# X-rayLaser/Implementing-JPEG-compression

Hardware: AMD Instinct MI355X
Metric: M 8x8 blocks/sec (DCT+quant+zigzag) (higher is better)
Workload: dtype f32

## Files before the change

implementing-jpeg-compression_amd/csrc/jpegx_entropy_decode.h:

```cpp
#pragma once
#include <hip/hip_runtime.h>
#include <stddef.h>
#include <stdint.h>

namespace jpegx_decode {
int levels_for(long long nblocks);
size_t phase1_bytes(size_t nbytes);
size_t phase2_bytes(size_t ncand, long long nblocks);
void enqueue_phase1(const uint8_t *d_bytes, size_t nbytes, void *d_ws1, hipStream_t st);
void enqueue_phase2(const uint8_t *d_bytes, size_t nbytes, long long nblocks, void *d_ws1, unsigned ncand, void *d_ws2,
                    int16_t *d_zz, hipStream_t st);

struct SegPlan {
    int seg, cmax, levels;
    int span_cap;
    unsigned nseg;
    size_t ws_bytes, state_bytes;
    bool ok;
    bool filter;
};
SegPlan seg_plan(size_t nbytes, long long nblocks, int level = 0, int filter = -1);
void enqueue_segmented(const uint8_t *d_bytes, size_t nbytes, long long nblocks, const SegPlan &plan, void *d_state, size_t state_cap, bool fresh, int parity,
                       void *d_ws, int16_t *d_zz, hipStream_t st);
}
```

implementing-jpeg-compression_amd/csrc/jpegx_entropy_decode.hip:

```cpp
#include <hip/hip_runtime.h>
#include <stdint.h>
#include <stdlib.h>

#include "../../include/jpegx.h"
#include "jpegx_entropy_decode.h"

namespace {

typedef unsigned u32x4 __attribute__((ext_vector_type(4)));
constexpr unsigned NIL = 0xFFFFFFFFu;
constexpr int CHUNK = 4096;
__device__ __forceinline__ int tile_off(int row, int chunk) { return row * 128 + ((chunk ^ (row & 7)) << 4); }

__device__ __forceinline__ unsigned zero_mask16(const unsigned char *__restrict__ bytes, size_t q0, size_t nbytes)
{
    unsigned m = 0;
    if (q0 + 16 <= nbytes) {
        const u32x4 v = *reinterpret_cast<const u32x4 *>(bytes + q0);
        const unsigned w[4] = {v.x, v.y, v.z, v.w};
#pragma unroll
        for (int k = 0; k < 16; ++k) m |= (((w[k >> 2] >> (8 * (k & 3))) & 0xFFu) == 0u ? 1u : 0u) << k;
    } else {
        for (int k = 0; k < 16; ++k)
            if (q0 + k < nbytes && bytes[q0 + k] == 0) m |= 1u << k;
    }
    return m;
}

__global__ __launch_bounds__(256) void k_dec_count(const unsigned char *__restrict__ bytes, size_t nbytes, unsigned *__restrict__ chunk_count)
{
    __shared__ unsigned part[4];
    const size_t q0 = (size_t)blockIdx.x * CHUNK + (size_t)threadIdx.x * 16;
    unsigned c = q0 < nbytes ? __popc(zero_mask16(bytes, q0, nbytes)) : 0u;
    if (blockIdx.x == 0 && threadIdx.x == 0) c += 1;
#pragma unroll
// ... 152 lines not shown

__device__ __forceinline__ void dec_blocks_body(const unsigned *__restrict__ words, size_t nbytes, const unsigned *__restrict__ start_pos,
                                                int nblk, int16_t *__restrict__ out, unsigned *__restrict__ head)
{
    __shared__ __attribute__((aligned(16))) unsigned char lds[64 * 128];
    const int lane = threadIdx.x, g0 = blockIdx.x * 64, g = g0 + lane;
#pragma unroll
    for (int c = 0; c < 8; ++c) *reinterpret_cast<u32x4 *>(lds + lane * 128 + c * 16) = u32x4{0u, 0u, 0u, 0u};
    __syncthreads();
    if (g < nblk) {
        const unsigned p = start_pos[g];
        const unsigned e = p == NIL ? NIL : parse_block<true>(words, (unsigned long long)nbytes * 8u, p, lds, lane);
        if (e == NIL) atomicOr(&head[1], 2u);
        else if (g == nblk - 1 && e != (unsigned)nbytes) atomicOr(&head[1], 4u);
    }
    __syncthreads();
    unsigned char *dst = reinterpret_cast<unsigned char *>(out) + (size_t)g0 * 128;
#pragma unroll
    for (int i = 0; i < 8; ++i) {
        const int row = i * 8 + (lane >> 3), c = lane & 7;
        const u32x4 q = *reinterpret_cast<const u32x4 *>(lds + tile_off(row, c));
        if (g0 + row < nblk) *reinterpret_cast<u32x4 *>(dst + (size_t)row * 128 + c * 16) = q;
    }
}

__global__ __launch_bounds__(64) void k_dec_blocks(const unsigned *__restrict__ words, size_t nbytes, const unsigned *__restrict__ start_pos,
                                                   int nblk, int16_t *__restrict__ out, unsigned *__restrict__ head)
{
    dec_blocks_body(words, nbytes, start_pos, nblk, out, head);
}

namespace seg {

typedef __attribute__((address_space(1))) unsigned gu32;
#define JPEGX_RLX_AGENT __ATOMIC_RELAXED, __HIP_MEMORY_SCOPE_AGENT

constexpr int REACH = 192;
constexpr int ROW = 144;
constexpr int FRONT = 16, TAIL = 208;
constexpr unsigned INVALID = 0xFFFFu, END = 0xFFFEu, AFTER = 0xFFFDu, POISON = 0xFFFCu, EXIT = 0x8000u;
constexpr unsigned TAG = 0x10000u;
constexpr unsigned SPIN_LIMIT = 1u << 18;
__device__ __forceinline__ bool is_exit(unsigned x) { return (x & EXIT) != 0 && x < POISON; }

struct Ws {
    unsigned *head;
    unsigned *next_head;
    unsigned *E;
    unsigned *C;
    unsigned *F;
    unsigned *wave_seg;
    u32x4 *prov;
    unsigned long long *trace;
};

__host__ __device__ inline size_t up16(size_t v) { return (v + 15) & ~(size_t)15; }

__host__ __device__ inline Ws carve(void *state, void *scratch, unsigned nseg, int cmax, long long nblocks, int parity, size_t *scratch_bytes = nullptr,
                                    size_t *state_bytes = nullptr)
{
    unsigned char *q = static_cast<unsigned char *>(state), *p = static_cast<unsigned char *>(scratch);
    Ws w;
    w.head = reinterpret_cast<unsigned *>(q + 64 * parity);
    w.next_head = reinterpret_cast<unsigned *>(q + 64 * (1 - parity));
    w.E = reinterpret_cast<unsigned *>(q + 128);
    if (state_bytes) *state_bytes = 128 + up16((size_t)nseg * 4);
    size_t o = 0;
    w.C = reinterpret_cast<unsigned *>(p + o); o += up16((size_t)nseg * 4 + 64);
    w.F = reinterpret_cast<unsigned *>(p + o); o += up16(((size_t)nseg + 1) * 4);
    w.wave_seg = reinterpret_cast<unsigned *>(p + o); o += up16((size_t)((nblocks + 63) / 64) * 4);
    w.prov = reinterpret_cast<u32x4 *>(p + o); o += up16((size_t)nseg * cmax * 16);
    w.trace = reinterpret_cast<unsigned long long *>(p + o);
#ifdef JPEGX_DECODE_STATS
    o += 64 + (size_t)nseg * 128;
#endif
    if (scratch_bytes) *scratch_bytes = o;
    return w;
}

__host__ __device__ inline int levels_of(int cmax)
{
    int l = 0;
    while ((1 << l) < cmax) ++l;
    return l;
}

__host__ __device__ inline size_t dec_lds_bytes(int span_cap) { return (size_t)span_cap + 64 * ROW + 1024 + 288; }

__host__ __device__ inline size_t lds_bytes(int seg, int cmax)
{
    return (size_t)(FRONT + seg + TAIL) + 64 * 12 + 256 + (size_t)cmax * (4 + levels_of(cmax));
}

constexpr int MARK_STEPS = 5;

__device__ __forceinline__ void fill_advance_table(unsigned char *tab, int lane)
{
    unsigned packed = 0;
#pragma unroll
// ... 76 lines not shown
    const size_t readable = (nbytes + 16) & ~(size_t)3;
    u32x4 v[PER];
#pragma unroll
    for (int k = 0; k < PER; ++k) {
        const int i = lane + THREADS * k;
        const long long off = first_off + 16LL * i;
        v[k] = u32x4{0u, 0u, 0u, 0u};
        if (i < npieces) {
            if (off >= 0 && (size_t)off + 16 <= readable) {
                v[k] = *reinterpret_cast<const u32x4 *>(bytes + off);
            } else {
                unsigned t[4] = {0u, 0u, 0u, 0u};
#pragma unroll
                for (int j = 0; j < 4; ++j) {
                    const long long o = off + 4 * j;
                    if (o >= 0 && (size_t)o + 4 <= readable) t[j] = *reinterpret_cast<const unsigned *>(bytes + o);
                }
                v[k] = u32x4{t[0], t[1], t[2], t[3]};
            }
        }
    }
#pragma unroll
    for (int k = 0; k < PER; ++k) {
        const int i = lane + THREADS * k;
        if (i < npieces) {
            u32x4 b = v[k];
            b.x = __builtin_bswap32(b.x); b.y = __builtin_bswap32(b.y); b.z = __builtin_bswap32(b.z); b.w = __builtin_bswap32(b.w);
            *reinterpret_cast<u32x4 *>(sm + 16 * i) = b;
        }
    }
}

__global__ __launch_bounds__(64) void k_seg_starts(const unsigned char *__restrict__ bytes, size_t nbytes, int seg, int cmax, unsigned nseg,
                                                   void *state, void *ws, long long nblocks, int parity, int filter)
{
    extern __shared__ __attribute__((aligned(16))) unsigned char sm[];
    const Ws W = carve(state, ws, nseg, cmax, nblocks, parity);
    gu32 *gE = (gu32 *)W.E;
    gu32 *ghead = (gu32 *)W.head;
    const int lane = threadIdx.x;
    const unsigned s = xcd_run_segment(blockIdx.x);
    if (s >= nseg) return;
#ifdef JPEGX_DECODE_STATS
    unsigned long long *trace = W.trace + 8 + (size_t)s * 16;
    if (lane == 0) trace[0] = wall_clock64();
    if (lane == 0 && s == 0) { unsigned *info = reinterpret_cast<unsigned *>(W.trace); info[4] = nseg; info[5] = (unsigned)seg; info[6] = (unsigned)cmax; info[7] = (unsigned)nblocks; }
#define JPEGX_PHASE(k) do { if (lane == 0) trace[(k) + 1] = wall_clock64(); } while (0)
#else
#define JPEGX_PHASE(k) do { } while (0)
#endif
    const int win = FRONT + seg + TAIL;
    const int levels = levels_of(cmax);
    unsigned *sw = reinterpret_cast<unsigned *>(sm);
    struct LaneRec { unsigned lo, hi, front; };
    LaneRec *rec = reinterpret_cast<LaneRec *>(sm + win);
    unsigned char *tab = reinterpret_cast<unsigned char *>(rec + 64);
    unsigned short *cpos = reinterpret_cast<unsigned short *>(tab + 256);
    unsigned short *J = cpos + cmax;
    unsigned char *Jk = reinterpret_cast<unsigned char *>(J + cmax) - cmax;

    const size_t base = (size_t)s * seg;
    stage_pieces<5>(bytes, nbytes, (long long)base - FRONT, win / 16, sm, lane);
    fill_advance_table(tab, lane);
    __syncthreads();
    JPEGX_PHASE(0);

    const int stretch = seg >> 6;
    const unsigned inv = ((1u << 20) + (unsigned)stretch - 1u) / (unsigned)stretch;
    const int p0 = lane * stretch;
    unsigned long long m;
    {
        const unsigned *swl = reinterpret_cast<const unsigned *>(sm + FRONT + p0);
// ... 20 lines not shown
        }
    }
    const unsigned mine = (unsigned)__popcll(m);
    unsigned incl = mine;
#pragma unroll
    for (int d = 1; d < 64; d <<= 1) {
        const unsigned u = (unsigned)__shfl_up((int)incl, d);
        if (lane >= d) incl += u;
    }
    const unsigned total = (unsigned)__shfl((int)incl, 63);
    rec[lane] = LaneRec{(unsigned)m, (unsigned)(m >> 32), incl - mine};
    const bool overflow = total > (unsigned)cmax;
    if (!overflow) {
        unsigned at = incl - mine;
        unsigned long long mm = m;
        while (mm) {
            const int i = __ffsll((long long)mm) - 1;
            mm &= mm - 1;
            cpos[at++] = (unsigned short)(p0 + i);
        }
    }
    __syncthreads();
    auto rank_of = [&](unsigned p, bool &is_cand) -> unsigned {
        const unsigned L = (p * inv) >> 20;
        const unsigned bit = p - L * (unsigned)stretch;
        const LaneRec r = rec[L];
        const unsigned long long mk = ((unsigned long long)r.hi << 32) | r.lo;
        is_cand = ((mk >> bit) & 1ull) != 0;
        return r.front + (unsigned)__popcll(mk & ((1ull << bit) - 1ull));
    };
    JPEGX_PHASE(1);

    bool poisoned = overflow;
    if (overflow && lane == 0) __hip_atomic_fetch_or(ghead + 2, 1u, JPEGX_RLX_AGENT);
    const size_t win_end = nbytes - base + FRONT;
    const unsigned end_bits = (unsigned)((win_end < (size_t)(win - 16) ? win_end : (size_t)(win - 16)) * 8u);
    unsigned nent = 0;
    bool konst = false;
    int lv = 1;
    while ((1u << (lv - 1)) < total && lv < levels) ++lv;
    auto chase = [&](unsigned c, unsigned &blocks) -> unsigned {
        unsigned cur = c, cnt = 0;
        for (int k = lv - 1; k >= 1; --k) {
            const unsigned nxt = Jk[k * cmax + cur];
            if (nxt != 0xFFu) { cur = nxt; cnt += 1u << k; }
        }
        const unsigned nxt0 = J[cur];
        if (nxt0 < EXIT) { cur = nxt0; cnt += 1u; }
        blocks = cnt + 1u;
        return J[cur];
    };
    unsigned my_exit_if_entry = INVALID, my_blocks_if_entry = 0;
    unsigned marks[2][3] = {{0u, 0u, 0u}, {0u, 0u, 0u}};
    if (!poisoned) {
        for (unsigned c0 = 0; c0 < total; c0 += 64) {
            const unsigned c = c0 + lane;
            const bool have = c < total;
            const unsigned p = have ? cpos[c] : 0u;
            unsigned mk[3];
            const unsigned e = parse_tab(sw, tab, (FRONT + p) * 8u, end_bits, have, mk);
#pragma unroll
            for (int k = 0; k < 3; ++k) {
                if (c0 == 0) marks[0][k] = mk[k];
                if (c0 == 64) marks[1][k] = mk[k];
            }
            unsigned code = INVALID;
            if (e != NIL) {
// ... 3 lines not shown
                else {
                    bool is_cand;
                    const unsigned i = rank_of(er, is_cand);
                    code = is_cand ? i : INVALID;
                }
            }
            if (have) J[c] = (unsigned short)code;
        }
        __syncthreads();
        JPEGX_PHASE(2);
        for (int k = 1; k < lv; ++k) {
            for (unsigned c = lane; c < total; c += 64) {
                unsigned two = 0xFFu;
                if (k == 1) {
                    const unsigned a = J[c];
                    if (a < EXIT) { const unsigned b = J[a]; if (b < EXIT) two = b; }
                } else {
                    const unsigned a = Jk[(k - 1) * cmax + c];
                    if (a != 0xFFu) two = Jk[(k - 1) * cmax + a];
                }
                Jk[k * cmax + c] = (unsigned char)two;
            }
            __syncthreads();
        }
        bool dummy_b;
        nent = total ? rank_of(REACH + 1, dummy_b) : 0u;
        if ((unsigned)lane < nent) my_exit_if_entry = chase((unsigned)lane, my_blocks_if_entry);
        if (nent >= 1 && nent <= 64) {
            const unsigned x = my_exit_if_entry;
            const unsigned long long valid = __ballot(x != INVALID);
            if (valid) {
                const unsigned x0 = (unsigned)__shfl((int)x, __ffsll((long long)valid) - 1);
                konst = __ballot(x != INVALID && x != x0) == 0;
                if (konst && lane == 0) __hip_atomic_store(gE + s, TAG | x0, JPEGX_RLX_AGENT);
            }
        }
    }
    JPEGX_PHASE(3);

    unsigned entry = INVALID, myexit = INVALID, count = 0, err = 0;
    if (!poisoned) {
        if (s == 0) {
            entry = total ? 0u : INVALID;
        } else {
            unsigned x = 0;
            unsigned dbg_spins = 0;
            for (unsigned spins = 0;;) {
                x = __hip_atomic_load(gE + (s - 1), JPEGX_RLX_AGENT);
                if (x != 0) break;
                ++dbg_spins;
                if (++spins > SPIN_LIMIT) { poisoned = true; break; }
                __builtin_amdgcn_s_sleep(2);
            }
            x &= 0xFFFFu;
            (void)dbg_spins;
#ifdef JPEGX_DECODE_STATS
            if (lane == 0) trace[12] = dbg_spins;
#endif
            if (poisoned || x == POISON) poisoned = true;
            else if (x == END || x == AFTER) entry = AFTER;
            else if (is_exit(x)) {
                const unsigned rel = x & 0x7FFFu;
                bool is_cand = false;
                const unsigned i = rel < (unsigned)seg ? rank_of(rel, is_cand) : 0u;
                entry = is_cand ? i : INVALID;
            }
        }
    }
    JPEGX_PHASE(4);
    if (!poisoned) {
        if (entry == AFTER) myexit = AFTER;
        else if (entry == INVALID) err |= filter ? 0x100u : 2u;
        else {
            if (entry < 64u && entry < nent) {
                myexit = (unsigned)__shfl((int)my_exit_if_entry, (int)entry);
                count = (unsigned)__shfl((int)my_blocks_if_entry, (int)entry);
            } else {
                myexit = chase(entry, count);
            }
            if (myexit == INVALID) { err |= filter ? 0x100u : 2u; count = 0; }
        }
        if ((err & 0xFFu) && lane == 0) __hip_atomic_fetch_or(ghead + 1, err & 0xFFu, JPEGX_RLX_AGENT);
        if ((err & 0x100u) && lane == 0) __hip_atomic_fetch_or(ghead + 2, 4u, JPEGX_RLX_AGENT);
        for (unsigned r0 = 0; r0 < count; r0 += 64) {
            const unsigned r = r0 + lane;
            unsigned cur = entry;
            if (r < count) {
                if (r & 1u) cur = J[cur];
                for (int k = 1; k < lv; ++k)
                    if ((r >> k) & 1u) cur = Jk[k * cmax + cur];
            }
            unsigned mk[3];
#pragma unroll
            for (int k = 0; k < 3; ++k) {
                const unsigned a = (unsigned)__shfl((int)marks[0][k], (int)(cur & 63u)), b = (unsigned)__shfl((int)marks[1][k], (int)(cur & 63u));
                mk[k] = cur < 64u ? a : (cur < 128u ? b : 0u);
            }
            if (r < count) W.prov[(size_t)s * cmax + r] = u32x4{(unsigned)base + cpos[cur], mk[0], mk[1], mk[2]};
        }
    } else if (lane == 0) {
        __hip_atomic_fetch_or(ghead + 2, 2u, JPEGX_RLX_AGENT);
    }
    if (lane == 0) {
        if (poisoned) __hip_atomic_store(gE + s, TAG | POISON, JPEGX_RLX_AGENT);
        else if (!konst || myexit == INVALID) __hip_atomic_store(gE + s, TAG | myexit, JPEGX_RLX_AGENT);
        W.C[s] = count;
    }
#ifdef JPEGX_DECODE_STATS
    if (lane == 0) { trace[15] = total; trace[13] = konst ? 1 : 0; trace[14] = count; }
#endif
    JPEGX_PHASE(5);
}

__global__ __launch_bounds__(1024) void k_seg_scan(unsigned nseg, int cmax, void *state, void *ws, long long nblocks, int parity)
{
    __shared__ unsigned carry[16];
    __shared__ unsigned base_s;
    const Ws W = carve(state, ws, nseg, cmax, nblocks, parity);
    const int t = threadIdx.x, lane = t & 63, wv = t >> 6;
    const unsigned nwaves = (unsigned)((nblocks + 63) / 64);
    if (t == 0) base_s = 0;
    __syncthreads();
    for (unsigned c0 = 0; c0 < nseg; c0 += 16384u) {
        const unsigned i0 = c0 + (unsigned)t * 16u;
        unsigned c[16];
        if (i0 + 16u <= nseg) {
#pragma unroll
            for (int k = 0; k < 4; ++k) {
                const u32x4 v = *reinterpret_cast<const u32x4 *>(W.C + i0 + 4 * k);
                c[4 * k] = v.x; c[4 * k + 1] = v.y; c[4 * k + 2] = v.z; c[4 * k + 3] = v.w;
            }
        } else {
#pragma unroll
            for (int k = 0; k < 16; ++k) c[k] = i0 + k < nseg ? W.C[i0 + k] : 0u;
        }
        unsigned sum = 0;
#pragma unroll
        for (int k = 0; k < 16; ++k) sum += c[k];
        unsigned incl = sum;
#pragma unroll
        for (int d = 1; d < 64; d <<= 1) {
            const unsigned u = (unsigned)__shfl_up((int)incl, d);
            if (lane >= d) incl += u;
        }
        if (lane == 63) carry[wv] = incl;
        __syncthreads();
        unsigned run = base_s + incl - sum;
        for (int k = 0; k < wv; ++k) run += carry[k];
#pragma unroll
        for (int k = 0; k < 16; ++k) {
            const unsigned i = i0 + k;
            if (i < nseg) {
                W.F[i] = run;
                for (unsigned m = (run + 63u) & ~63u; m < run + c[k]; m += 64)
                    if ((m >> 6) < nwaves) W.wave_seg[m >> 6] = i;
            }
            run += c[k];
        }
        __syncthreads();
        if (t == 1023) base_s = run;
        __syncthreads();
    }
    if (t == 0) {
        const unsigned run = base_s;
        W.F[nseg] = run;
        W.head[3] = run;
        unsigned err = 0;
        if ((long long)run < nblocks) err |= 1u;
        if ((long long)run > nblocks) err |= 4u;
        if (err) atomicOr(&W.head[1], err);
    }
}

__global__ __launch_bounds__(256) void k_dec_blocks_lds(const unsigned char *__restrict__ bytes, size_t nbytes, unsigned nseg, int cmax, void *state,
                                                        const void *ws, int nblk, int span_cap, int16_t *__restrict__ out, int parity)
{
    extern __shared__ __attribute__((aligned(16))) unsigned char sm[];
    const Ws W = carve(state, const_cast<void *>(ws), nseg, cmax, nblk, parity);
    for (unsigned i = blockIdx.x * 256u + threadIdx.x; i < nseg; i += gridDim.x * 256u) W.E[i] = 0u;
    if (blockIdx.x == 0 && threadIdx.x < 16) W.next_head[threadIdx.x] = 0u;
    const unsigned s0 = W.wave_seg[blockIdx.x], refused = W.head[1], handed_on = W.head[2];
    if (refused != 0 || handed_on != 0) return;
    const int t = threadIdx.x, lane = t & 63, part = t >> 6;
    const int tile_idx = blockIdx.x, g0 = tile_idx * 64, g = g0 + lane;
#ifdef JPEGX_DECODE_STATS
    unsigned long long *trace3 = W.trace + 8 + (size_t)tile_idx * 16;
    if (t == 0 && (unsigned)tile_idx < nseg) trace3[7] = wall_clock64();
#define JPEGX_PHASE3(k) do { if (t == 0 && (unsigned)tile_idx < nseg) trace3[k] = wall_clock64(); } while (0)
#else
#define JPEGX_PHASE3(k) do { } while (0)
#endif
    unsigned char *tile = sm + span_cap;
    unsigned char *dummy = tile + 64 * ROW + t * 4;
    unsigned *Fs = reinterpret_cast<unsigned *>(tile + 64 * ROW + 1024);
    for (int i = t; i < 64 * ROW / 16; i += 256) *reinterpret_cast<u32x4 *>(tile + i * 16) = u32x4{0u, 0u, 0u, 0u};
    if (t <= 64) Fs[t] = s0 + t <= nseg ? W.F[s0 + t] : 0xFFFFFFFFu;
    __syncthreads();
    auto entry_of = [&](unsigned blk) -> u32x4 {
        unsigned lo = 0, hi = 65;
        while (hi - lo > 1) {
            const unsigned mid = (lo + hi) >> 1;
            if (Fs[mid] <= blk) lo = mid; else hi = mid;
        }
        unsigned sgm = s0 + lo, first = Fs[lo];
        if (lo == 64) {
            unsigned a = s0 + 64, b = nseg;
            while (b - a > 1) {
                const unsigned mid = a + ((b - a) >> 1);
                if (W.F[mid] <= blk) a = mid; else b = mid;
            }
            sgm = a; first = W.F[a];
        }
        return W.prov[(size_t)sgm * cmax + (blk - first)];
// ... 74 lines not shown
    const char *force = getenv("JPEGX_DECODE_SEG");
    if (force && *force) k = atoi(force) / 256;
    if (level >= 1) k = 1;
    k = k < 1 ? 1 : (k > 16 ? 16 : k);
    if (level == 0 && !(force && *force)) {
        static const int ncu = [] { int v = 0, dev = 0; if (hipGetDevice(&dev) != hipSuccess || hipDeviceGetAttribute(&v, hipDeviceAttributeMultiprocessorCount, dev) != hipSuccess || v <= 0) v = 256; return v; }();
        const int cmax_l0 = p.filter ? 96 : 128;
        auto margin = [&](int kk) {
            const size_t lds = (seg::lds_bytes(256 * kk, cmax_l0) + 1279) / 1280 * 1280;
            const size_t per_cu = 163840 / lds > 32 ? 32 : 163840 / lds;
            const double slots = (double)ncu * (double)per_cu, waves = (double)((nbytes + 256 * (size_t)kk - 1) / (256 * (size_t)kk));
            return 1.0 - waves / slots;
        };
        if (margin(k) < 0.03) {
            int best = k;
            double best_margin = 0.03;
            for (int kk : {k + 1, k - 1, k + 2, k - 2})
                if (kk >= 1 && kk <= 16 && per_byte * 256.0 * kk <= 56.0 && margin(kk) > best_margin) { best = kk; best_margin = margin(kk); }
            k = best;
        }
    }
    p.seg = 256 * k;
    p.cmax = p.filter ? 96 : 128;
    const char *fc = getenv("JPEGX_DECODE_CMAX");
    if (fc && *fc) { p.cmax = atoi(fc); p.cmax = p.cmax < 32 ? 32 : (p.cmax > 128 ? 128 : p.cmax); }
    p.levels = seg::levels_of(p.cmax);
    p.nseg = (unsigned)((nbytes + p.seg - 1) / p.seg);
    size_t span = (size_t)(per_block * 64.0 * 1.5) + 64;
    span = (span + 15) & ~(size_t)15;
    if (span < 1024) span = 1024;
    if (span > 64 * 185 + 48) span = 64 * 185 + 48;
    p.span_cap = (int)span;
    p.ok = nbytes > 0 && (size_t)p.nseg * p.cmax * 16 <= ((size_t)1 << 32) && nblocks > 0;
    seg::carve(nullptr, nullptr, p.nseg ? p.nseg : 1, p.cmax, nblocks > 0 ? nblocks : 1, 0, &p.ws_bytes, &p.state_bytes);
    return p;
}

void enqueue_segmented(const uint8_t *d_bytes, size_t nbytes, long long nblocks, const SegPlan &p, void *d_state, size_t state_cap, bool fresh, int parity,
                       void *d_ws, int16_t *d_zz, hipStream_t st)
{
    if (fresh) (void)hipMemsetAsync(d_state, 0, state_cap, st);
#ifdef JPEGX_DECODE_STATS
    (void)hipMemsetAsync(d_ws, 0, p.ws_bytes, st);
#endif
    const unsigned run8 = 8u << seg::RUN_LOG;
    hipLaunchKernelGGL(seg::k_seg_starts, dim3((p.nseg + run8 - 1) / run8 * run8), dim3(64), seg::lds_bytes(p.seg, p.cmax), st, d_bytes, nbytes, p.seg, p.cmax,
                       p.nseg, d_state, d_ws, nblocks, parity, p.filter ? 1 : 0);
    hipLaunchKernelGGL(seg::k_seg_scan, dim3(1), dim3(1024), 0, st, p.nseg, p.cmax, d_state, d_ws, nblocks, parity);
    hipLaunchKernelGGL(seg::k_dec_blocks_lds, dim3((unsigned)((nblocks + 63) / 64)), dim3(256), seg::dec_lds_bytes(p.span_cap), st, d_bytes, nbytes,
                       p.nseg, p.cmax, d_state, d_ws, (int)nblocks, p.span_cap, d_zz, parity);
}

size_t phase1_bytes(size_t nbytes) { return 64 + ((nbytes + CHUNK - 1) / CHUNK + 1) * 4; }

size_t phase2_bytes(size_t ncand, long long nblocks)
{
    return ((size_t)ncand * 4 + 15) / 16 * 16 + (size_t)levels_for(nblocks) * ncand * 4 + (size_t)nblocks * 4 + 64;
}

void enqueue_phase1(const uint8_t *d_bytes, size_t nbytes, void *d_ws1, hipStream_t st)
{
    unsigned *head = static_cast<unsigned *>(d_ws1);
    unsigned *chunk = head + 4;
    const int nchunks = (int)((nbytes + CHUNK - 1) / CHUNK);
    (void)hipMemsetAsync(head, 0, 16, st);
    hipLaunchKernelGGL(k_dec_count, dim3(nchunks), dim3(256), 0, st, d_bytes, nbytes, chunk);
    hipLaunchKernelGGL(k_dec_scan, dim3(1), dim3(1024), 0, st, chunk, nchunks, head);
}

void enqueue_phase2(const uint8_t *d_bytes, size_t nbytes, long long nblocks, void *d_ws1, unsigned ncand, void *d_ws2,
                    int16_t *d_zz, hipStream_t st)
{
    unsigned *head = static_cast<unsigned *>(d_ws1);
    unsigned *chunk = head + 4;
    unsigned *cand_pos = static_cast<unsigned *>(d_ws2);
    unsigned *J = cand_pos + ((size_t)ncand * 4 + 15) / 16 * 4;
    const int levels = levels_for(nblocks);
    unsigned *start_pos = J + (size_t)levels * ncand;
    const unsigned *words = reinterpret_cast<const unsigned *>(d_bytes);
    const int nchunks = (int)((nbytes + CHUNK - 1) / CHUNK);
    const unsigned gc = (ncand + 255) / 256;
    hipLaunchKernelGGL(k_dec_scatter, dim3(nchunks), dim3(256), 0, st, d_bytes, nbytes, chunk, cand_pos);
    hipLaunchKernelGGL(k_dec_parse, dim3(gc), dim3(256), 0, st, words, nbytes, cand_pos, ncand, J);
// ... 9 lines not shown
```

implementing-jpeg-compression_amd/csrc/jpegx_hostpipe.cpp:

```cpp
#include <hip/hip_runtime.h>
#include <stdint.h>
#include <stdio.h>
#include <stdlib.h>
#include <string.h>
#include <time.h>
#include <sys/mman.h>

#include <atomic>
#include <functional>
#include <mutex>
#include <thread>
#include <vector>

#include "../../include/jpegx.h"
#include "jpegx_entropy_decode.h"

extern "C" void jpegx_internal_set_error(const char *msg);
extern "C" int jpegx_internal_forward_u8_sized(const uint8_t *d_in, int H, int W, ptrdiff_t pitch, int bs, int mode, double param, unsigned flags,
                                               int16_t *d_out, unsigned *block_bytes, unsigned *wave_bytes, unsigned *half_info, jpegx_stream_t stream);
extern "C" void jpegx_internal_entropy_views(void *d_workspace, long long nblocks, unsigned **block_bytes, unsigned **wave_bytes, unsigned **half_info);
extern "C" int jpegx_internal_entropy_emit2(const int16_t *d_zz, long long nblocks, const void *d_workspace, uint8_t *d_out, jpegx_stream_t stream);
extern "C" int jpegx_internal_entropy_scan(long long nblocks, void *d_workspace, jpegx_stream_t stream);

namespace {
// ... 17 lines not shown
    } while (0)

struct Span {
    void *p = nullptr;
    size_t cap = 0;
    bool pinned = false;
    int ensure(size_t bytes)
    {
        if (bytes <= cap) return JPEGX_OK;
        if (p) {
            if (pinned) (void)hipHostFree(p); else (void)hipFree(p);
            p = nullptr;
            cap = 0;
        }
        const size_t want = bytes + bytes / 8 + 4096;
        if (pinned) HP_TRY(hipHostMalloc(&p, want, hipHostMallocDefault)); else HP_TRY(hipMalloc(&p, want));
        cap = want;
        return JPEGX_OK;
    }
    void release()
    {
        if (p) { if (pinned) (void)hipHostFree(p); else (void)hipFree(p); }
        p = nullptr;
        cap = 0;
    }
};

constexpr int MAX_DEVICES = 16;
constexpr int MAX_BANDS = JPEGX_MAX_IMAGE_BANDS;

struct BandSlot {
    Span d_in, d_zz, d_ws, d_out, d_tmp;
    Span d_seg, d_seg_state;
    void *seg_clean = nullptr;
    size_t seg_clean_cap = 0;
    unsigned seg_calls = 0;
    int seg_parity = -1;
    bool sized = false;
    unsigned filter_pause = 0;
    bool last_filter = false;
};

struct DevicePool {
    std::mutex mu;
    hipStream_t stream = nullptr;
    hipStream_t aux[2] = {nullptr, nullptr};
    hipEvent_t ev[MAX_BANDS] = {};
    hipEvent_t ev_x = nullptr;
    BandSlot slot[MAX_BANDS];
    Span d_packed;
    Span h_in{nullptr, 0, true}, h_out{nullptr, 0, true}, h_head{nullptr, 0, true};
    bool open = false;
    size_t out_bytes = 0;
};

constexpr int POOL_CONTEXTS = 4;
DevicePool g_pool[MAX_DEVICES][POOL_CONTEXTS];

thread_local DevicePool *t_held = nullptr;
thread_local int t_held_device = -1;

int lock_pool(DevicePool **out)
{
    int dev = 0;
    HP_TRY(hipGetDevice(&dev));
    if (dev < 0 || dev >= MAX_DEVICES) return fail(JPEGX_E_UNSUPPORTED, "device index beyond the pool table");
    if (t_held != nullptr)
        return fail(JPEGX_E_INVALID, t_held->open ? "a compress job is open on this thread: finish or abort it first"
                                                   : "this thread already holds a device pool");
    DevicePool *pool = nullptr;
// ... 396 lines not shown
{
    if (!h_planes) return fail(JPEGX_E_INVALID, "null pointer");
    return compress_image_impl(h_planes, nullptr, nbands, elem_size, H, W, pitch, bs, mode, param, prefix, prefix_len, length_prefixes, alloc, user, nbytes);
}

int jpegx_host_compress_image_packed(const uint8_t *h_pixels, int nbands, int H, int W, ptrdiff_t pitch, int bs,
                                     int mode, double param, const void *prefix, size_t prefix_len, int length_prefixes,
                                     jpegx_alloc_fn alloc, void *user, size_t *nbytes)
{
    if (!h_pixels) return fail(JPEGX_E_INVALID, "null pointer");
    return compress_image_impl(nullptr, h_pixels, nbands, 1, H, W, pitch, bs, mode, param, prefix, prefix_len, length_prefixes, alloc, user, nbytes);
}

}

namespace {
constexpr int DECODE_RETRY_GENERAL = 1;

thread_local int t_last_decode_level = -1;

int decode_on_device(BandSlot &slot, size_t nbytes, long long nblocks, hipStream_t st, int level)
{
    int rc;
    if ((rc = slot.d_zz.ensure((size_t)nblocks * 128))) return rc;
    const char *force = getenv("JPEGX_DECODE_GENERAL");
    if (force && *force && *force != '0') level = 2;
    if (level == 1 && jpegx_decode::seg_plan(nbytes, nblocks, 0).seg == 256) level = 2;
    const jpegx_decode::SegPlan plan = jpegx_decode::seg_plan(nbytes, nblocks, level, (level == 0 && slot.filter_pause > 0) ? 0 : -1);
    if (level == 0 && slot.filter_pause > 0) --slot.filter_pause;
    slot.last_filter = plan.filter;
    t_last_decode_level = level;
    if (level < 2 && plan.ok) {
        if ((rc = slot.d_seg.ensure(plan.ws_bytes)) || (rc = slot.d_seg_state.ensure(plan.state_bytes))) return rc;
        bool fresh = slot.d_seg_state.p != slot.seg_clean || slot.d_seg_state.cap != slot.seg_clean_cap;
        if (const char *ff = getenv("JPEGX_DECODE_FRESH")) fresh = fresh || (*ff && *ff != '0');
        slot.seg_clean = slot.d_seg_state.p;
        slot.seg_clean_cap = slot.d_seg_state.cap;
        slot.seg_parity = (int)(slot.seg_calls++ & 1u);
        jpegx_decode::enqueue_segmented(static_cast<const uint8_t *>(slot.d_in.p), nbytes, nblocks, plan, slot.d_seg_state.p, slot.d_seg_state.cap, fresh,
                                        slot.seg_parity, slot.d_seg.p, static_cast<int16_t *>(slot.d_zz.p), st);
        HP_TRY(hipGetLastError());
        return JPEGX_OK;
    }
    slot.seg_parity = -1;
    if ((rc = slot.d_ws.ensure(jpegx_decode::phase1_bytes(nbytes)))) return rc;
    jpegx_decode::enqueue_phase1(static_cast<const uint8_t *>(slot.d_in.p), nbytes, slot.d_ws.p, st);
    unsigned head[4] = {0, 0, 0, 0};
    HP_TRY(hipMemcpyAsync(head, slot.d_ws.p, 16, hipMemcpyDeviceToHost, st));
    HP_TRY(hipStreamSynchronize(st));
    const unsigned ncand = head[0];
    if (ncand == 0 || (long long)ncand < nblocks) return fail(JPEGX_E_INVALID, "entropy stream holds fewer blocks than the plane has");
    if ((rc = slot.d_tmp.ensure(jpegx_decode::phase2_bytes(ncand, nblocks)))) return rc;
    jpegx_decode::enqueue_phase2(static_cast<const uint8_t *>(slot.d_in.p), nbytes, nblocks, slot.d_ws.p, ncand, slot.d_tmp.p,
                                 static_cast<int16_t *>(slot.d_zz.p), st);
    HP_TRY(hipGetLastError());
    return JPEGX_OK;
}

int decode_status(BandSlot &slot)
{
    unsigned head[16] = {0};
    const bool seg = slot.seg_parity >= 0;
    const unsigned char *src = seg ? static_cast<const unsigned char *>(slot.d_seg_state.p) + 64 * slot.seg_parity : static_cast<const unsigned char *>(slot.d_ws.p);
    HP_TRY(hipMemcpy(head, src, 64, hipMemcpyDeviceToHost));
    if (const char *dump = getenv("JPEGX_DECODE_STATS")) {
        if (seg) {
            std::vector<unsigned char> raw(slot.d_seg.cap);
            HP_TRY(hipMemcpy(raw.data(), slot.d_seg.p, raw.size(), hipMemcpyDeviceToHost));
            if (FILE *f = fopen(dump, "wb")) { fwrite(raw.data(), 1, raw.size(), f); fclose(f); }
        }
    }
    if (seg && head[2] != 0) {
        if ((head[2] & 4u) && slot.last_filter) slot.filter_pause = 64;
        return DECODE_RETRY_GENERAL;
    }
    if (head[1] != 0) return fail(JPEGX_E_INVALID, "entropy stream is not a sequence of well-formed blocks (device decoder)");
    return JPEGX_OK;
}

int check_decompress_shape(const uint8_t *h_bytes, size_t nbytes, int H, int W, int bs)
{
    if (!h_bytes) return fail(JPEGX_E_INVALID, "null host pointer");
    if (H <= 0 || W <= 0 || (H % 8) || (W % 8)) return fail(JPEGX_E_INVALID, "plane height and width must be positive multiples of 8");
    if ((long long)(H / 8) * (W / 8) > 0x7FFFFFC0LL) return fail(JPEGX_E_INVALID, "block count must be in 1 .. 2^31-64");
    if (bs < 1 || bs > 255) return fail(JPEGX_E_UNSUPPORTED, "host_decompress supports block_size 1..255");
    if (nbytes == 0 || nbytes >= 0xFFFFFFF0ull) return fail(JPEGX_E_INVALID, "entropy stream empty or beyond 4 GiB");
    return JPEGX_OK;
}

int enqueue_back(BandSlot &slot, const uint8_t *h_bytes, size_t nbytes, int H, int W, int bs, int mode, double param,
                 ptrdiff_t dev_pitch, hipStream_t st, int level)
{
    const long long nblocks = (long long)(H / 8) * (W / 8);
    int rc;
    if ((rc = slot.d_in.ensure(nbytes + 16)) || (rc = slot.d_out.ensure((size_t)H * bs * dev_pitch))) return rc;
    HP_TRY(hipMemsetAsync(static_cast<uint8_t *>(slot.d_in.p) + (nbytes & ~(size_t)3), 0, 16 + (nbytes & 3), st));
// ... 160 lines not shown
    for (int level = 0; level < 2; ++level)
        for (int filter = -1; filter <= 0; ++filter) {
            const jpegx_decode::SegPlan p = jpegx_decode::seg_plan(nbytes, nblocks, level, filter);
            if (p.state_bytes > m) m = p.state_bytes;
        }
    return (m + 255) & ~(size_t)255;
}
}

extern "C" size_t jpegx_entropy_decode_workspace_bytes(size_t nbytes, long long nblocks)
{
    if (nbytes == 0 || nblocks <= 0) return 0;
    size_t scratch = 0;
    for (int level = 0; level < 2; ++level)
        for (int filter = -1; filter <= 0; ++filter) {
            const jpegx_decode::SegPlan p = jpegx_decode::seg_plan(nbytes, nblocks, level, filter);
            if (p.ws_bytes > scratch) scratch = p.ws_bytes;
        }
    return decode_state_span(nbytes, nblocks) + scratch + 256;
}

extern "C" int jpegx_entropy_decode(const uint8_t *d_bytes, size_t nbytes, long long nblocks, void *d_workspace, int16_t *d_zz,
                                    int level, jpegx_stream_t stream)
{
    if (!d_bytes || !d_workspace || !d_zz) return fail(JPEGX_E_INVALID, "null device pointer");
    if (nblocks <= 0 || nblocks > 0x7FFFFFC0LL) return fail(JPEGX_E_INVALID, "block count must be in 1 .. 2^31-64");
    if (nbytes == 0 || nbytes >= 0xFFFFFFF0ull) return fail(JPEGX_E_INVALID, "entropy stream empty or beyond 4 GiB");
    if (level < 0 || level > 1) return fail(JPEGX_E_UNSUPPORTED, "levels 0 and 1 run on caller buffers; the whole-stream scheme is jpegx_host_entropy_decode_gpu's");
    if ((reinterpret_cast<uintptr_t>(d_workspace) & 255u) != 0) return fail(JPEGX_E_INVALID, "workspace must be 256-byte aligned");
    const jpegx_decode::SegPlan plan = jpegx_decode::seg_plan(nbytes, nblocks, level);
    if (!plan.ok) return fail(JPEGX_E_UNSUPPORTED, "stream too long for the segmented decoder");
    const size_t state_span = decode_state_span(nbytes, nblocks);
    unsigned char *w = static_cast<unsigned char *>(d_workspace);
    jpegx_decode::enqueue_segmented(d_bytes, nbytes, nblocks, plan, w, state_span, true, 0, w + state_span, d_zz, (hipStream_t)stream);
    HP_TRY(hipGetLastError());
    return JPEGX_OK;
}

extern "C" int jpegx_entropy_decode_status(const void *d_workspace, jpegx_stream_t stream)
{
    if (!d_workspace) return fail(JPEGX_E_INVALID, "null device pointer");
    unsigned head[16] = {0};
    HP_TRY(hipMemcpyAsync(head, d_workspace, 64, hipMemcpyDeviceToHost, (hipStream_t)stream));
    HP_TRY(hipStreamSynchronize((hipStream_t)stream));
    if (head[2] != 0) return 1;
    if (head[1] != 0) return fail(JPEGX_E_INVALID, "entropy stream is not a sequence of well-formed blocks (device decoder)");
    return JPEGX_OK;
}

int jpegx_host_entropy_decode_gpu(const uint8_t *h_bytes, size_t nbytes, long long nblocks, int16_t *h_zz)
{
    if (!h_bytes || !h_zz) return fail(JPEGX_E_INVALID, "null host pointer");
    if (nblocks <= 0 || nblocks > 0x7FFFFFC0LL) return fail(JPEGX_E_INVALID, "block count must be in 1 .. 2^31-64");
    if (nbytes == 0 || nbytes >= 0xFFFFFFF0ull) return fail(JPEGX_E_INVALID, "entropy stream empty or beyond 4 GiB");
    PoolLock lock;
    if (lock.rc) return lock.rc;
    DevicePool *pool = lock.pool;
    int rc;
    if ((rc = ensure_streams(pool, false))) return rc;
    hipStream_t st = pool->stream;
    BandSlot &slot = pool->slot[0];
    if ((rc = slot.d_in.ensure(nbytes + 16))) return rc;
    HP_TRY(hipMemsetAsync(static_cast<uint8_t *>(slot.d_in.p) + (nbytes & ~(size_t)3), 0, 16 + (nbytes & 3), st));
    HP_TRY(hipMemcpyAsync(slot.d_in.p, h_bytes, nbytes, hipMemcpyHostToDevice, st));
    for (int level = 0; level < 3; ++level) {
        if ((rc = decode_on_device(slot, nbytes, nblocks, st, level))) return rc;
        HP_TRY(hipMemcpyAsync(h_zz, slot.d_zz.p, (size_t)nblocks * 128, hipMemcpyDeviceToHost, st));
// ... 7 lines not shown
{
    DevicePool *pool = nullptr;
    int rc = lock_pool(&pool);
    if (rc) return rc;
    if ((rc = ensure_streams(pool, false)) || (rc = pool->slot[0].d_in.ensure(in_bytes ? in_bytes : 1)) ||
        (rc = pool->slot[0].d_out.ensure(out_bytes ? out_bytes : 1))) {
        unlock_pool(pool);
        return rc;
    }
    *d_in = pool->slot[0].d_in.p;
    *d_out = pool->slot[0].d_out.p;
    *stream = pool->stream;
    return JPEGX_OK;
}

void jpegx_internal_pool_release(void)
{
    if (t_held && !t_held->open) unlock_pool(t_held);
}

int jpegx_host_pool_release(void)
{
    int dev = 0;
    HP_TRY(hipGetDevice(&dev));
    if (dev < 0 || dev >= MAX_DEVICES) return fail(JPEGX_E_UNSUPPORTED, "device index beyond the pool table");
    if (t_held != nullptr)
        return fail(JPEGX_E_INVALID, t_held->open ? "a compress job is open on this thread: finish or abort it first"
                                                   : "this thread already holds a device pool");
    for (DevicePool &ctx : g_pool[dev]) {
        std::lock_guard<std::mutex> guard(ctx.mu);
        DevicePool *pool = &ctx;
        for (BandSlot &b : pool->slot) {
            for (Span *s : {&b.d_in, &b.d_zz, &b.d_ws, &b.d_out, &b.d_tmp, &b.d_seg, &b.d_seg_state}) s->release();
            b.seg_clean = nullptr;
            b.seg_clean_cap = 0;
            b.filter_pause = 0;
            b.last_filter = false;
        }
        for (Span *s : {&pool->d_packed, &pool->h_in, &pool->h_out, &pool->h_head}) s->release();
        if (pool->stream) { (void)hipStreamDestroy(pool->stream); pool->stream = nullptr; }
        for (hipStream_t &s : pool->aux)
            if (s) { (void)hipStreamDestroy(s); s = nullptr; }
        for (hipEvent_t &e : pool->ev)
            if (e) { (void)hipEventDestroy(e); e = nullptr; }
        if (pool->ev_x) { (void)hipEventDestroy(pool->ev_x); pool->ev_x = nullptr; }
    }
    return JPEGX_OK;
}

}
```

Before: 16970.

## Replace per-call state memset and parity buffers with per-call tokens in segmented decoder

Segment exit records become 64-bit words tagged with a per-call token, so successor segments wait until the token matches instead of waiting for a nonzero value. This removes the memset of decode state on fresh calls, the in-kernel clearing of E and the next head, and the parity double-buffering. Error and handoff flags no longer go through global atomic ORs on the head. They are packed into the upper bits of the per-segment count and reduced in the scan kernel, which writes the whole head in one store. The cost is wider atomics and a host-side token counter, and it assumes segment counts fit in 16 bits.

New measurement: 16950, median of 3. Within noise of the previous version (-0.1%).

```diff
diff --git a/implementing-jpeg-compression_amd/csrc/jpegx_entropy_decode.h b/implementing-jpeg-compression_amd/csrc/jpegx_entropy_decode.h
--- a/implementing-jpeg-compression_amd/csrc/jpegx_entropy_decode.h
+++ b/implementing-jpeg-compression_amd/csrc/jpegx_entropy_decode.h
@@ -20,6 +20,6 @@
     bool filter;
 };
 SegPlan seg_plan(size_t nbytes, long long nblocks, int level = 0, int filter = -1);
-void enqueue_segmented(const uint8_t *d_bytes, size_t nbytes, long long nblocks, const SegPlan &plan, void *d_state, size_t state_cap, bool fresh, int parity,
-                       void *d_ws, int16_t *d_zz, hipStream_t st);
+void enqueue_segmented(const uint8_t *d_bytes, size_t nbytes, long long nblocks, const SegPlan &plan, void *d_state, void *d_ws, int16_t *d_zz,
+                       hipStream_t st);
 }
diff --git a/implementing-jpeg-compression_amd/csrc/jpegx_entropy_decode.hip b/implementing-jpeg-compression_amd/csrc/jpegx_entropy_decode.hip
--- a/implementing-jpeg-compression_amd/csrc/jpegx_entropy_decode.hip
+++ b/implementing-jpeg-compression_amd/csrc/jpegx_entropy_decode.hip
@@ -1,6 +1,10 @@
 #include <hip/hip_runtime.h>
 #include <stdint.h>
 #include <stdlib.h>
+#include <unistd.h>
+
+#include <atomic>
+#include <chrono>
 
 #include "../../include/jpegx.h"
 #include "jpegx_entropy_decode.h"
@@ -219,21 +223,20 @@
 
 namespace seg {
 
-typedef __attribute__((address_space(1))) unsigned gu32;
+typedef __attribute__((address_space(1))) unsigned long long gu64;
 #define JPEGX_RLX_AGENT __ATOMIC_RELAXED, __HIP_MEMORY_SCOPE_AGENT
 
 constexpr int REACH = 192;
 constexpr int ROW = 144;
 constexpr int FRONT = 16, TAIL = 208;
 constexpr unsigned INVALID = 0xFFFFu, END = 0xFFFEu, AFTER = 0xFFFDu, POISON = 0xFFFCu, EXIT = 0x8000u;
-constexpr unsigned TAG = 0x10000u;
+constexpr int TOKEN_SHIFT = 16;
 constexpr unsigned SPIN_LIMIT = 1u << 18;
 __device__ __forceinline__ bool is_exit(unsigned x) { return (x & EXIT) != 0 && x < POISON; }
 
 struct Ws {
     unsigned *head;
-    unsigned *next_head;
-    unsigned *E;
+    unsigned long long *E;
     unsigned *C;
     unsigned *F;
     unsigned *wave_seg;
@@ -243,15 +246,14 @@
 
 __host__ __device__ inline size_t up16(size_t v) { return (v + 15) & ~(size_t)15; }
 
-__host__ __device__ inline Ws carve(void *state, void *scratch, unsigned nseg, int cmax, long long nblocks, int parity, size_t *scratch_bytes = nullptr,
+__host__ __device__ inline Ws carve(void *state, void *scratch, unsigned nseg, int cmax, long long nblocks, size_t *scratch_bytes = nullptr,
                                     size_t *state_bytes = nullptr)
 {
     unsigned char *q = static_cast<unsigned char *>(state), *p = static_cast<unsigned char *>(scratch);
     Ws w;
-    w.head = reinterpret_cast<unsigned *>(q + 64 * parity);
-    w.next_head = reinterpret_cast<unsigned *>(q + 64 * (1 - parity));
-    w.E = reinterpret_cast<unsigned *>(q + 128);
-    if (state_bytes) *state_bytes = 128 + up16((size_t)nseg * 4);
+    w.head = reinterpret_cast<unsigned *>(q);
+    w.E = reinterpret_cast<unsigned long long *>(q + 64);
+    if (state_bytes) *state_bytes = 64 + up16((size_t)nseg * 8);
     size_t o = 0;
     w.C = reinterpret_cast<unsigned *>(p + o); o += up16((size_t)nseg * 4 + 64);
     w.F = reinterpret_cast<unsigned *>(p + o); o += up16(((size_t)nseg + 1) * 4);
@@ -394,12 +396,12 @@
 }
 
 __global__ __launch_bounds__(64) void k_seg_starts(const unsigned char *__restrict__ bytes, size_t nbytes, int seg, int cmax, unsigned nseg,
-                                                   void *state, void *ws, long long nblocks, int parity, int filter)
+                                                   void *state, void *ws, long long nblocks, unsigned long long token, int filter)
 {
     extern __shared__ __attribute__((aligned(16))) unsigned char sm[];
-    const Ws W = carve(state, ws, nseg, cmax, nblocks, parity);
-    gu32 *gE = (gu32 *)W.E;
-    gu32 *ghead = (gu32 *)W.head;
+    const Ws W = carve(state, ws, nseg, cmax, nblocks);
+    gu64 *gE = (gu64 *)W.E;
+    const unsigned long long tok = token << TOKEN_SHIFT;
     const int lane = threadIdx.x;
     const unsigned s = xcd_run_segment(blockIdx.x);
     if (s >= nseg) return;
@@ -486,7 +488,7 @@
     JPEGX_PHASE(1);
 
     bool poisoned = overflow;
-    if (overflow && lane == 0) __hip_atomic_fetch_or(ghead + 2, 1u, JPEGX_RLX_AGENT);
+    unsigned handoff = overflow ? 1u : 0u;
     const size_t win_end = nbytes - base + FRONT;
     const unsigned end_bits = (unsigned)((win_end < (size_t)(win - 16) ? win_end : (size_t)(win - 16)) * 8u);
     unsigned nent = 0;
@@ -556,7 +558,7 @@
             if (valid) {
                 const unsigned x0 = (unsigned)__shfl((int)x, __ffsll((long long)valid) - 1);
                 konst = __ballot(x != INVALID && x != x0) == 0;
-                if (konst && lane == 0) __hip_atomic_store(gE + s, TAG | x0, JPEGX_RLX_AGENT);
+                if (konst && lane == 0) __hip_atomic_store(gE + s, tok | x0, JPEGX_RLX_AGENT);
             }
         }
     }
@@ -567,16 +569,16 @@
         if (s == 0) {
             entry = total ? 0u : INVALID;
         } else {
-            unsigned x = 0;
+            unsigned long long xw = 0;
             unsigned dbg_spins = 0;
             for (unsigned spins = 0;;) {
-                x = __hip_atomic_load(gE + (s - 1), JPEGX_RLX_AGENT);
-                if (x != 0) break;
+                xw = __hip_atomic_load(gE + (s - 1), JPEGX_RLX_AGENT);
+                if ((xw >> TOKEN_SHIFT) == token) break;
                 ++dbg_spins;
                 if (++spins > SPIN_LIMIT) { poisoned = true; break; }
                 __builtin_amdgcn_s_sleep(2);
             }
-            x &= 0xFFFFu;
+            const unsigned x = (unsigned)xw & 0xFFFFu;
             (void)dbg_spins;
 #ifdef JPEGX_DECODE_STATS
             if (lane == 0) trace[12] = dbg_spins;
@@ -604,8 +606,7 @@
             }
             if (myexit == INVALID) { err |= filter ? 0x100u : 2u; count = 0; }
         }
-        if ((err & 0xFFu) && lane == 0) __hip_atomic_fetch_or(ghead + 1, err & 0xFFu, JPEGX_RLX_AGENT);
-        if ((err & 0x100u) && lane == 0) __hip_atomic_fetch_or(ghead + 2, 4u, JPEGX_RLX_AGENT);
+        if (err & 0x100u) handoff |= 4u;
         for (unsigned r0 = 0; r0 < count; r0 += 64) {
             const unsigned r = r0 + lane;
             unsigned cur = entry;
@@ -622,13 +623,13 @@
             }
             if (r < count) W.prov[(size_t)s * cmax + r] = u32x4{(unsigned)base + cpos[cur], mk[0], mk[1], mk[2]};
         }
-    } else if (lane == 0) {
-        __hip_atomic_fetch_or(ghead + 2, 2u, JPEGX_RLX_AGENT);
+    } else {
+        handoff |= 2u;
     }
     if (lane == 0) {
-        if (poisoned) __hip_atomic_store(gE + s, TAG | POISON, JPEGX_RLX_AGENT);
-        else if (!konst || myexit == INVALID) __hip_atomic_store(gE + s, TAG | myexit, JPEGX_RLX_AGENT);
-        W.C[s] = count;
+        if (poisoned) __hip_atomic_store(gE + s, tok | POISON, JPEGX_RLX_AGENT);
+        else if (!konst || myexit == INVALID) __hip_atomic_store(gE + s, tok | myexit, JPEGX_RLX_AGENT);
+        W.C[s] = count | ((err & 0xFFu) << 16) | (handoff << 24);
     }
 #ifdef JPEGX_DECODE_STATS
     if (lane == 0) { trace[15] = total; trace[13] = konst ? 1 : 0; trace[14] = count; }
@@ -636,14 +637,14 @@
     JPEGX_PHASE(5);
 }
 
-__global__ __launch_bounds__(1024) void k_seg_scan(unsigned nseg, int cmax, void *state, void *ws, long long nblocks, int parity)
+__global__ __launch_bounds__(1024) void k_seg_scan(unsigned nseg, int cmax, void *state, void *ws, long long nblocks)
 {
     __shared__ unsigned carry[16];
-    __shared__ unsigned base_s;
-    const Ws W = carve(state, ws, nseg, cmax, nblocks, parity);
+    __shared__ unsigned base_s, flags_s;
+    const Ws W = carve(state, ws, nseg, cmax, nblocks);
     const int t = threadIdx.x, lane = t & 63, wv = t >> 6;
     const unsigned nwaves = (unsigned)((nblocks + 63) / 64);
-    if (t == 0) base_s = 0;
+    if (t == 0) { base_s = 0; flags_s = 0; }
     __syncthreads();
     for (unsigned c0 = 0; c0 < nseg; c0 += 16384u) {
         const unsigned i0 = c0 + (unsigned)t * 16u;
@@ -658,9 +659,10 @@
 #pragma unroll
             for (int k = 0; k < 16; ++k) c[k] = i0 + k < nseg ? W.C[i0 + k] : 0u;
         }
-        unsigned sum = 0;
-#pragma unroll
-        for (int k = 0; k < 16; ++k) sum += c[k];
+        unsigned sum = 0, flags = 0;
+#pragma unroll
+        for (int k = 0; k < 16; ++k) { flags |= c[k] >> 16; c[k] &= 0xFFFFu; sum += c[k]; }
+        if (flags) atomicOr(&flags_s, flags);
         unsigned incl = sum;
 #pragma unroll
         for (int d = 1; d < 64; d <<= 1) {
@@ -686,23 +688,20 @@
         __syncthreads();
     }
     if (t == 0) {
-        const unsigned run = base_s;
+        const unsigned run = base_s, flags = flags_s;
         W.F[nseg] = run;
-        W.head[3] = run;
-        unsigned err = 0;
+        unsigned err = flags & 0xFFu;
         if ((long long)run < nblocks) err |= 1u;
         if ((long long)run > nblocks) err |= 4u;
-        if (err) atomicOr(&W.head[1], err);
+        *reinterpret_cast<u32x4 *>(W.head) = u32x4{0u, err, flags >> 8, run};
     }
 }
 
 __global__ __launch_bounds__(256) void k_dec_blocks_lds(const unsigned char *__restrict__ bytes, size_t nbytes, unsigned nseg, int cmax, void *state,
-                                                        const void *ws, int nblk, int span_cap, int16_t *__restrict__ out, int parity)
+                                                        const void *ws, int nblk, int span_cap, int16_t *__restrict__ out)
 {
     extern __shared__ __attribute__((aligned(16))) unsigned char sm[];
-    const Ws W = carve(state, const_cast<void *>(ws), nseg, cmax, nblk, parity);
-    for (unsigned i = blockIdx.x * 256u + threadIdx.x; i < nseg; i += gridDim.x * 256u) W.E[i] = 0u;
-    if (blockIdx.x == 0 && threadIdx.x < 16) W.next_head[threadIdx.x] = 0u;
+    const Ws W = carve(state, const_cast<void *>(ws), nseg, cmax, nblk);
     const unsigned s0 = W.wave_seg[blockIdx.x], refused = W.head[1], handed_on = W.head[2];
     if (refused != 0 || handed_on != 0) return;
     const int t = threadIdx.x, lane = t & 63, part = t >> 6;
@@ -843,23 +842,39 @@
     if (span > 64 * 185 + 48) span = 64 * 185 + 48;
     p.span_cap = (int)span;
     p.ok = nbytes > 0 && (size_t)p.nseg * p.cmax * 16 <= ((size_t)1 << 32) && nblocks > 0;
-    seg::carve(nullptr, nullptr, p.nseg ? p.nseg : 1, p.cmax, nblocks > 0 ? nblocks : 1, 0, &p.ws_bytes, &p.state_bytes);
+    seg::carve(nullptr, nullptr, p.nseg ? p.nseg : 1, p.cmax, nblocks > 0 ? nblocks : 1, &p.ws_bytes, &p.state_bytes);
     return p;
 }
 
-void enqueue_segmented(const uint8_t *d_bytes, size_t nbytes, long long nblocks, const SegPlan &p, void *d_state, size_t state_cap, bool fresh, int parity,
-                       void *d_ws, int16_t *d_zz, hipStream_t st)
-{
-    if (fresh) (void)hipMemsetAsync(d_state, 0, state_cap, st);
+unsigned long long next_call_token()
+{
+    static std::atomic<unsigned long long> counter{[] {
+        unsigned long long x = (unsigned long long)std::chrono::steady_clock::now().time_since_epoch().count() ^
+                               ((unsigned long long)getpid() << 32) ^ (unsigned long long)(uintptr_t)&counter;
+        x += 0x9E3779B97F4A7C15ull;
+        x = (x ^ (x >> 30)) * 0xBF58476D1CE4E5B9ull;
+        x = (x ^ (x >> 27)) * 0x94D049BB133111EBull;
+        return x ^ (x >> 31);
+    }()};
+    for (;;) {
+        const unsigned long long t = counter.fetch_add(1, std::memory_order_relaxed) & 0xFFFFFFFFFFFFull;
+        if (t != 0) return t;
+    }
+}
+
+void enqueue_segmented(const uint8_t *d_bytes, size_t nbytes, long long nblocks, const SegPlan &p, void *d_state, void *d_ws, int16_t *d_zz,
+                       hipStream_t st)
+{
+    const unsigned long long token = next_call_token();
 #ifdef JPEGX_DECODE_STATS
     (void)hipMemsetAsync(d_ws, 0, p.ws_bytes, st);
 #endif
     const unsigned run8 = 8u << seg::RUN_LOG;
     hipLaunchKernelGGL(seg::k_seg_starts, dim3((p.nseg + run8 - 1) / run8 * run8), dim3(64), seg::lds_bytes(p.seg, p.cmax), st, d_bytes, nbytes, p.seg, p.cmax,
-                       p.nseg, d_state, d_ws, nblocks, parity, p.filter ? 1 : 0);
-    hipLaunchKernelGGL(seg::k_seg_scan, dim3(1), dim3(1024), 0, st, p.nseg, p.cmax, d_state, d_ws, nblocks, parity);
+                       p.nseg, d_state, d_ws, nblocks, token, p.filter ? 1 : 0);
+    hipLaunchKernelGGL(seg::k_seg_scan, dim3(1), dim3(1024), 0, st, p.nseg, p.cmax, d_state, d_ws, nblocks);
     hipLaunchKernelGGL(seg::k_dec_blocks_lds, dim3((unsigned)((nblocks + 63) / 64)), dim3(256), seg::dec_lds_bytes(p.span_cap), st, d_bytes, nbytes,
-                       p.nseg, p.cmax, d_state, d_ws, (int)nblocks, p.span_cap, d_zz, parity);
+                       p.nseg, p.cmax, d_state, d_ws, (int)nblocks, p.span_cap, d_zz);
 }
 
 size_t phase1_bytes(size_t nbytes) { return 64 + ((nbytes + CHUNK - 1) / CHUNK + 1) * 4; }
diff --git a/implementing-jpeg-compression_amd/csrc/jpegx_hostpipe.cpp b/implementing-jpeg-compression_amd/csrc/jpegx_hostpipe.cpp
--- a/implementing-jpeg-compression_amd/csrc/jpegx_hostpipe.cpp
+++ b/implementing-jpeg-compression_amd/csrc/jpegx_hostpipe.cpp
@@ -73,10 +73,7 @@
 struct BandSlot {
     Span d_in, d_zz, d_ws, d_out, d_tmp;
     Span d_seg, d_seg_state;
-    void *seg_clean = nullptr;
-    size_t seg_clean_cap = 0;
-    unsigned seg_calls = 0;
-    int seg_parity = -1;
+    bool seg_ran = false;
     bool sized = false;
     unsigned filter_pause = 0;
     bool last_filter = false;
@@ -539,17 +536,13 @@
     t_last_decode_level = level;
     if (level < 2 && plan.ok) {
         if ((rc = slot.d_seg.ensure(plan.ws_bytes)) || (rc = slot.d_seg_state.ensure(plan.state_bytes))) return rc;
-        bool fresh = slot.d_seg_state.p != slot.seg_clean || slot.d_seg_state.cap != slot.seg_clean_cap;
-        if (const char *ff = getenv("JPEGX_DECODE_FRESH")) fresh = fresh || (*ff && *ff != '0');
-        slot.seg_clean = slot.d_seg_state.p;
-        slot.seg_clean_cap = slot.d_seg_state.cap;
-        slot.seg_parity = (int)(slot.seg_calls++ & 1u);
-        jpegx_decode::enqueue_segmented(static_cast<const uint8_t *>(slot.d_in.p), nbytes, nblocks, plan, slot.d_seg_state.p, slot.d_seg_state.cap, fresh,
-                                        slot.seg_parity, slot.d_seg.p, static_cast<int16_t *>(slot.d_zz.p), st);
+        slot.seg_ran = true;
+        jpegx_decode::enqueue_segmented(static_cast<const uint8_t *>(slot.d_in.p), nbytes, nblocks, plan, slot.d_seg_state.p, slot.d_seg.p,
+                                        static_cast<int16_t *>(slot.d_zz.p), st);
         HP_TRY(hipGetLastError());
         return JPEGX_OK;
     }
-    slot.seg_parity = -1;
+    slot.seg_ran = false;
     if ((rc = slot.d_ws.ensure(jpegx_decode::phase1_bytes(nbytes)))) return rc;
     jpegx_decode::enqueue_phase1(static_cast<const uint8_t *>(slot.d_in.p), nbytes, slot.d_ws.p, st);
     unsigned head[4] = {0, 0, 0, 0};
@@ -567,8 +560,8 @@
 int decode_status(BandSlot &slot)
 {
     unsigned head[16] = {0};
-    const bool seg = slot.seg_parity >= 0;
-    const unsigned char *src = seg ? static_cast<const unsigned char *>(slot.d_seg_state.p) + 64 * slot.seg_parity : static_cast<const unsigned char *>(slot.d_ws.p);
+    const bool seg = slot.seg_ran;
+    const unsigned char *src = static_cast<const unsigned char *>(seg ? slot.d_seg_state.p : slot.d_ws.p);
     HP_TRY(hipMemcpy(head, src, 64, hipMemcpyDeviceToHost));
     if (const char *dump = getenv("JPEGX_DECODE_STATS")) {
         if (seg) {
@@ -795,7 +788,7 @@
     if (!plan.ok) return fail(JPEGX_E_UNSUPPORTED, "stream too long for the segmented decoder");
     const size_t state_span = decode_state_span(nbytes, nblocks);
     unsigned char *w = static_cast<unsigned char *>(d_workspace);
-    jpegx_decode::enqueue_segmented(d_bytes, nbytes, nblocks, plan, w, state_span, true, 0, w + state_span, d_zz, (hipStream_t)stream);
+    jpegx_decode::enqueue_segmented(d_bytes, nbytes, nblocks, plan, w, w + state_span, d_zz, (hipStream_t)stream);
     HP_TRY(hipGetLastError());
     return JPEGX_OK;
 }
@@ -869,8 +862,7 @@
         DevicePool *pool = &ctx;
         for (BandSlot &b : pool->slot) {
             for (Span *s : {&b.d_in, &b.d_zz, &b.d_ws, &b.d_out, &b.d_tmp, &b.d_seg, &b.d_seg_state}) s->release();
-            b.seg_clean = nullptr;
-            b.seg_clean_cap = 0;
+            b.seg_ran = false;
             b.filter_pause = 0;
             b.last_filter = false;
         }
diff --git a/microbench/entropy_decode_calls.py b/microbench/entropy_decode_calls.py
--- /dev/null
+++ b/microbench/entropy_decode_calls.py
@@ -0,0 +1,62 @@
+#!/usr/bin/env python3
+import argparse
+import ctypes
+import json
+import os
+import sys
+
+import numpy as np
+
+REPO = os.path.dirname(os.path.dirname(os.path.abspath(__file__)))
+sys.path.insert(0, REPO)
+sys.path.insert(0, os.path.join(REPO, "implementing-jpeg-compression_amd"))
+import jpegx
+
+
+def main():
+    ap = argparse.ArgumentParser()
+    ap.add_argument("--calls", type=int, default=20)
+    args = ap.parse_args()
+    jpegx.require_device()
+    L = jpegx.lib()
+    n = 4096
+    blocks = (n // 8) ** 2
+    res = {}
+    for kind in ("noise", "smooth"):
+        src, zz = jpegx.DeviceBuffer(n * n * 4), jpegx.DeviceBuffer(blocks * 128)
+        jpegx.generate_plane_device(src.ptr, n, n, kind, seed=0, plane=0)
+        jpegx.forward_fused_device(src.ptr, n, n, zz.ptr, "qtable", 0.0, jpegx.F_PIXEL_INPUT)
+        ws = jpegx.DeviceBuffer(int(L.jpegx_entropy_workspace_bytes(blocks)))
+        jpegx.check(L.jpegx_entropy_sizes(zz.ptr, blocks, ws.ptr, None), "sizes")
+        tot = ctypes.c_ulonglong(0)
+        jpegx.check(L.jpegx_entropy_total(ws.ptr, ctypes.byref(tot), None), "total")
+        nbytes = int(tot.value)
+        coded = jpegx.DeviceBuffer(nbytes + 64)
+        jpegx.check(L.jpegx_memset(coded.ptr, 0, nbytes + 64, None), "memset")
+        jpegx.check(L.jpegx_entropy_emit(zz.ptr, blocks, ws.ptr, coded.ptr, None), "emit")
+        dws = jpegx.DeviceBuffer(int(L.jpegx_entropy_decode_workspace_bytes(nbytes, blocks)))
+        out = jpegx.DeviceBuffer(blocks * 128)
+
+        def call():
+            jpegx.check(L.jpegx_entropy_decode(coded.ptr, nbytes, blocks, dws.ptr, out.ptr, 0, None), "entropy_decode")
+        call()
+        jpegx.check(L.jpegx_entropy_decode_status(dws.ptr, None), "entropy_decode_status")
+        e0, e1 = jpegx.Event(), jpegx.Event()
+        e0.record()
+        for _ in range(args.calls):
+            call()
+        e1.record()
+        e1.synchronize()
+        us = e0.elapsed_ms(e1) * 1e3 / args.calls
+        jpegx.check(L.jpegx_entropy_decode_status(dws.ptr, None), "entropy_decode_status")
+        blob = coded.download((nbytes,), np.uint8).tobytes()
+        ok = bool(np.array_equal(out.download((blocks, 64), np.int16), jpegx.entropy_decode(blob, blocks)))
+        res[kind] = {"stream_bytes": nbytes, "calls": args.calls, "us_per_call": round(us, 1), "matches_host_parser": ok}
+        for b in (src, zz, ws, coded, dws, out):
+            b.free()
+    print(json.dumps(res))
+    return 0 if all(r["matches_host_parser"] for r in res.values()) else 1
+
+
+if __name__ == "__main__":
+    sys.exit(main())
```
